# sphereisaiahmin-dev/sph-pie

Hardware: AMD Instinct MI355X
Metric: feeds/sec + sessions scanned/sec, 10^8 synthetic sessions, 1/2/4/8 MI355X (higher is better)
Workload: dtype int64

## Files before the change

include/pie_scan.h:

```cpp
#ifndef PIE_SCAN_H
#define PIE_SCAN_H

#include <stddef.h>
#include <stdint.h>

#ifdef __cplusplus
extern "C" {
#endif

#define PIE_ABI_VERSION 1

enum {
    PIE_OK = 0,
    PIE_E_INVAL = -1,
    PIE_E_NODEVICE = -2,
    PIE_E_HIP = -3,
    PIE_E_NOMEM = -4,
    PIE_E_CAPACITY = -5,
    PIE_E_STATE = -6
};

#define PIE_GEN_INTERVAL  1u
#define PIE_GEN_CLUSTERED 2u
#define PIE_GEN_TIME_ORDERED 4u
// ... 77 lines not shown
    uint64_t mask;
} pie_query;
int pie_scan_batch_begin(pie_ctx *ctx, const pie_query *queries, int n_q);
int pie_scan_batch_finish(pie_ctx *ctx, size_t *m_out);
int pie_scan_batch(pie_ctx *ctx, const pie_query *queries, int n_q, size_t *m_out);
int pie_batch_union_device_ptrs(pie_ctx *ctx, void **uoff_dev , void **rows_dev ,
                                void **mask_lo_dev , void **mask_hi_dev ,
                                size_t *mu_out);
int pie_batch_read_union(pie_ctx *ctx, int64_t *uoff_out, int32_t *rows_out, uint64_t *masks_out, size_t cap, size_t *mu_out);
#define PIE_WIDE_MAX 512
int pie_scan_wide_begin(pie_ctx *ctx, const pie_query *queries, int n_q);
int pie_scan_wide_finish(pie_ctx *ctx, size_t *m_out, size_t m_cap, int *n_q_out);
int pie_batch_union_wide_device_ptrs(pie_ctx *ctx, void **uoff_dev , void **rows_dev ,
                                     void **masks_dev , int *words_out, size_t *mu_out);
int pie_batch_read_union_wide(pie_ctx *ctx, int64_t *uoff_out, int32_t *rows_out, uint64_t *masks_out , size_t cap,
                              int *words_out, size_t *mu_out);
int pie_batch_pack_union_wide_device(pie_ctx *ctx, void *dst_i32, size_t u_pad, size_t cap);
int pie_scan_wide_begin_union(pie_ctx *ctx, const pie_query *queries, int n_q, void *msg_i32, size_t u_pad, size_t cap);
int pie_scan_wide_finish_packed(pie_ctx *ctx, size_t *m_out, size_t m_cap, int *n_q_out, int *ready_out);
int pie_set_batch_lanes(pie_ctx *ctx, int n_lanes);
int pie_batch_lanes(pie_ctx *ctx);
int pie_batch_room(pie_ctx *ctx);
int pie_scan_batch_flush(pie_ctx *ctx);
int pie_scan_batch_begin_union(pie_ctx *ctx, const pie_query *queries, int n_q, void *msg_i32, size_t u_pad, size_t cap);
int pie_scan_batch_begin_packed(pie_ctx *ctx, const pie_query *queries, int n_q, void *msg_i32, size_t msg_stride_words,
                                size_t u_pad, size_t idx_cap, void *counts_i32, size_t counts_stride_words);
int pie_scan_batch_finish_packed(pie_ctx *ctx, size_t *m_out, int *ready_out);
int pie_batch_read_results(pie_ctx *ctx, int qi, int32_t *counts_out, int64_t *offsets_out, int32_t *idx_out, size_t idx_cap,
                           size_t *m_out);
int pie_batch_result_device_ptrs(pie_ctx *ctx, int qi, void **counts_dev, void **offsets_dev, void **idx_dev);
int pie_batch_pack_union_device(pie_ctx *ctx, void *dst_i32, size_t u_pad, size_t cap);
int pie_batch_read_user_feed(pie_ctx *ctx, int qi, int32_t user, int32_t *idx_out, size_t idx_cap, size_t *k_out);

int pie_batch_fetch_requests(pie_ctx *ctx, const int32_t *qi, const int32_t *user, size_t n_req, size_t cap_rows, int64_t *req_off_out,
                             int32_t *idx_out, int64_t *start_out, int64_t *end_out, int32_t *disc_out, size_t *total_out);

int pie_read_results(pie_ctx *ctx, int32_t *counts_out, int64_t *offsets_out, int32_t *idx_out, size_t idx_cap,
                     size_t *m_out);
int pie_read_user_feed(pie_ctx *ctx, int32_t user, int32_t *idx_out, size_t idx_cap, size_t *k_out);
int pie_result_device_ptrs(pie_ctx *ctx, void **counts_dev, void **offsets_dev, void **idx_dev);
int pie_copy_results_device(pie_ctx *ctx, void *counts_dst, void *offsets_dst, void *idx_dst, size_t idx_cap);
int pie_pack_results_device(pie_ctx *ctx, void *dst_i32, size_t u_pad, size_t idx_cap);
int pie_fetch_rows(pie_ctx *ctx, const int32_t *idx, size_t m, int64_t *start, int64_t *end, int32_t *user,
                   int32_t *disc);

int pie_expired_queue(pie_ctx *ctx, int64_t prev_now, int64_t now, int32_t *queue_out, size_t cap, size_t *q_out);
// ... 231 lines not shown
```

sph-pie_amd/binding.py:

```python
import ctypes as C
import os

import numpy as np

from .build import HIP_LIB

PIE_GEN_INTERVAL = 1
PIE_GEN_CLUSTERED = 2
PIE_GEN_TIME_ORDERED = 4
PIE_END_NONE = -(2 ** 63)
INT64_MIN = -(2 ** 63)

PIE_E_CAPACITY = -5
PIE_E_STATE = -6
PIE_COMPACT_SHRINK = 1


class PieError(RuntimeError):
    def __init__(self, code, text):
        super().__init__("pie_scan error %d: %s" % (code, text))
        self.code = code


class PieTableInfo(C.Structure):
# ... 49 lines not shown
    ("pie_delete_users", C.c_int, [_P, _P, C.c_size_t, _P, C.c_size_t, C.POINTER(C.c_size_t), _P]),
    ("pie_delete_users_plan", C.c_int, [_P, C.c_size_t, C.c_int32, _P, _P]),
    ("pie_prune_before", C.c_int, [_P, C.c_int64, _P, C.c_size_t, C.POINTER(C.c_size_t)]),
    ("pie_retention_purge", C.c_int, [_P, C.c_int64, C.c_int32, C.c_int64, _P, C.c_size_t, C.POINTER(C.c_size_t)]),
    ("pie_retention_purge_tz", C.c_int, [_P, C.c_int64, C.c_int32, _P, _P, C.c_int32, _P, C.c_size_t, C.POINTER(C.c_size_t)]),
    ("pie_append_rows", C.c_int, [_P, _P, _P, _P, _P, C.c_size_t, C.c_int32]),
    ("pie_set_disciplines", C.c_int, [_P, C.c_uint64, C.c_int32]),
    ("pie_scan", C.c_int, [_P, C.c_int64, C.c_int64, _P, _P, _P, C.c_size_t, C.POINTER(C.c_size_t)]),
    ("pie_scan_device", C.c_int, [_P, C.c_int64, C.c_int64, C.POINTER(C.c_size_t)]),
    ("pie_scan_begin", C.c_int, [_P, C.c_int64, C.c_int64]),
    ("pie_scan_finish", C.c_int, [_P, C.POINTER(C.c_size_t)]),
    ("pie_scan_begin_packed", C.c_int, [_P, C.c_int64, C.c_int64, C.c_void_p, C.c_size_t, C.c_size_t]),
    ("pie_scan_finish_packed", C.c_int, [_P, C.POINTER(C.c_size_t), C.POINTER(C.c_int)]),
    ("pie_scan_begin_packed2", C.c_int, [_P, C.c_int64, C.c_int64, C.c_void_p, C.c_size_t, C.c_size_t, C.c_void_p]),
    ("pie_host_alloc", C.c_int, [_P, C.c_size_t, C.POINTER(_P), C.POINTER(_P)]),
    ("pie_host_free", C.c_int, [_P, _P]),
    ("pie_set_scan_form", C.c_int, [_P, C.c_int]),
    ("pie_set_ordered_run", C.c_int, [_P, C.c_int]),
    ("pie_set_wide_ordered", C.c_int, [_P, C.c_int]),
    ("pie_set_batch_lanes", C.c_int, [_P, C.c_int]),
    ("pie_batch_lanes", C.c_int, [_P]),
    ("pie_batch_room", C.c_int, [_P]),
    ("pie_scan_batch_flush", C.c_int, [_P]),
    ("pie_batch_pack_union_device", C.c_int, [_P, _P, C.c_size_t, C.c_size_t]),
    ("pie_table_info_get", C.c_int, [_P, C.POINTER(PieTableInfo)]),
    ("pie_hot_layout", C.c_int, [_P, _P, C.POINTER(C.c_int64), _P, _P, _P, C.c_size_t, _P, C.c_size_t]),
    ("pie_hot_order_key", C.c_uint64, [C.c_uint32, C.c_int32, C.c_uint32]),
    ("pie_hot_slot_bits", C.c_uint32, [C.c_uint32]),
    ("pie_scan_batch_begin", C.c_int, [_P, C.POINTER(PieQuery), C.c_int]),
    ("pie_scan_batch_finish", C.c_int, [_P, C.POINTER(C.c_size_t)]),
    ("pie_scan_batch", C.c_int, [_P, C.POINTER(PieQuery), C.c_int, C.POINTER(C.c_size_t)]),
    ("pie_scan_batch_begin_union", C.c_int, [_P, C.POINTER(PieQuery), C.c_int, C.c_void_p, C.c_size_t, C.c_size_t]),
    ("pie_batch_union_device_ptrs", C.c_int, [_P, C.POINTER(_P), C.POINTER(_P), C.POINTER(_P), C.POINTER(_P), C.POINTER(C.c_size_t)]),
    ("pie_batch_read_union", C.c_int, [_P, _P, _P, _P, C.c_size_t, C.POINTER(C.c_size_t)]),
    ("pie_scan_batch_begin_packed", C.c_int, [_P, C.POINTER(PieQuery), C.c_int, C.c_void_p, C.c_size_t, C.c_size_t, C.c_size_t, C.c_void_p, C.c_size_t]),
    ("pie_scan_batch_finish_packed", C.c_int, [_P, C.POINTER(C.c_size_t), C.POINTER(C.c_int)]),
    ("pie_scan_wide_begin", C.c_int, [_P, C.POINTER(PieQuery), C.c_int]),
    ("pie_scan_wide_finish", C.c_int, [_P, _P, C.c_size_t, C.POINTER(C.c_int)]),
    ("pie_batch_union_wide_device_ptrs", C.c_int, [_P, C.POINTER(_P), C.POINTER(_P), C.POINTER(_P), C.POINTER(C.c_int), C.POINTER(C.c_size_t)]),
    ("pie_batch_read_union_wide", C.c_int, [_P, _P, _P, _P, C.c_size_t, C.POINTER(C.c_int), C.POINTER(C.c_size_t)]),
    ("pie_batch_pack_union_wide_device", C.c_int, [_P, _P, C.c_size_t, C.c_size_t]),
    ("pie_scan_wide_begin_union", C.c_int, [_P, C.POINTER(PieQuery), C.c_int, _P, C.c_size_t, C.c_size_t]),
    ("pie_scan_wide_finish_packed", C.c_int, [_P, _P, C.c_size_t, C.POINTER(C.c_int), C.POINTER(C.c_int)]),
    ("pie_batch_mask_codes", C.c_int, [C.POINTER(PieQuery), C.c_int, _P, C.c_int32, _P, _P, _P, C.c_size_t, _P, _P]),
    ("pie_batch_read_results", C.c_int, [_P, C.c_int, _P, _P, _P, C.c_size_t, C.POINTER(C.c_size_t)]),
    ("pie_batch_result_device_ptrs", C.c_int, [_P, C.c_int, C.POINTER(_P), C.POINTER(_P), C.POINTER(_P)]),
# ... 379 lines not shown

    def scan_finish_packed(self):
        m, ready = C.c_size_t(0), C.c_int(0)
        rc = self._lib.pie_scan_finish_packed(self._ctx, C.byref(m), C.byref(ready))
        if self._begun and rc != -6:
            self._begun.pop(0)
        self._check(rc)
        return int(m.value), bool(ready.value)

    def scan_pipelined(self, k, now, cutoff):
        m = 0
        if k <= 0:
            return m
        self.scan_begin(now, cutoff)
        for i in range(k):
            if i + 1 < k:
                self.scan_begin(now, cutoff)
            m = self.scan_finish()
        return m

    _q_cache = None

    @staticmethod
    def _queries(queries):
        hit = PieScan._q_cache
        if hit is not None and hit[2] is queries and len(queries) == len(hit[0]):
            return hit[1]
        key = tuple(queries)
        if hit is not None and hit[0] == key:
            return hit[1]
        arr = (PieQuery * len(queries))()
        for k, (now, cutoff, mask) in enumerate(queries):
            arr[k].now, arr[k].cutoff, arr[k].mask = int(now), int(cutoff), int(mask) & (2 ** 64 - 1)
        PieScan._q_cache = (key, arr, queries)
        return arr

    def scan_batch_begin(self, queries):
        arr = self._queries(queries)
        self._check(self._lib.pie_scan_batch_begin(self._ctx, arr, len(queries)))
        self._batches = getattr(self, "_batches", [])
        self._batches.append(len(queries))

    def scan_batch_begin_packed(self, queries, msg_ptr, msg_stride, u_pad, idx_cap, counts_ptr=None, counts_stride=0):
        arr = self._queries(queries)
        self._check(self._lib.pie_scan_batch_begin_packed(self._ctx, arr, len(queries), msg_ptr, int(msg_stride), int(u_pad),
                                                          int(idx_cap), counts_ptr, int(counts_stride)))
        self._batches = getattr(self, "_batches", [])
        self._batches.append(len(queries))

    def scan_batch_begin_union(self, queries, msg_ptr, u_pad, cap):
        arr = self._queries(queries)
# ... 130 lines not shown
            if rc == PIE_E_CAPACITY and cap_rows is None and total.value > cap:
                cap = int(total.value)
                continue
            self._check(rc)
            break
        t = total.value
        return off, idx[:t], start[:t], end[:t], disc[:t]

    def batch_result_device_ptrs(self, qi):
        a, b, c = _P(), _P(), _P()
        self._check(self._lib.pie_batch_result_device_ptrs(self._ctx, int(qi), C.byref(a), C.byref(b), C.byref(c)))
        return a.value, b.value, c.value

    def set_batch_lanes(self, n_lanes):
        self._check(self._lib.pie_set_batch_lanes(self._ctx, int(n_lanes)))

    def batch_lanes(self):
        return int(self._lib.pie_batch_lanes(self._ctx))

    def batch_room(self):
        return int(self._lib.pie_batch_room(self._ctx))

    def scan_batch_pipelined(self, k, queries, depth=3):
        ms, begun, done = [], 0, 0
        depth = depth * self.batch_lanes()
        room = self._lib.pie_batch_room
        while done < k:
            while begun < k and begun - done < depth and room(self._ctx) > 0:
                self.scan_batch_begin(queries)
                begun += 1
                if begun == k:
                    self._check(self._lib.pie_scan_batch_flush(self._ctx))
            ms = self.scan_batch_finish()
            done += 1
        return ms

    def scan_batch_flush(self):
        self._check(self._lib.pie_scan_batch_flush(self._ctx))

    def result_device_ptrs(self):
        a, b, c = _P(), _P(), _P()
        self._check(self._lib.pie_result_device_ptrs(self._ctx, C.byref(a), C.byref(b), C.byref(c)))
        return a.value, b.value, c.value

    def copy_results_device(self, counts_ptr=None, offsets_ptr=None, idx_ptr=None, idx_cap=0):
        self._check(self._lib.pie_copy_results_device(self._ctx, counts_ptr, offsets_ptr, idx_ptr, int(idx_cap)))

    def pack_results_device(self, dst_ptr, u_pad, idx_cap):
        self._check(self._lib.pie_pack_results_device(self._ctx, dst_ptr, int(u_pad), int(idx_cap)))

    def fetch_rows(self, idx):
        idx = _col(idx, np.int32)
        m = idx.shape[0]
        s, e = np.empty(m, np.int64), np.empty(m, np.int64)
        u, d = np.empty(m, np.int32), np.empty(m, np.int32)
        self._check(self._lib.pie_fetch_rows(self._ctx, _ptr(idx), m, _ptr(s), _ptr(e), _ptr(u), _ptr(d)))
        return s, e, u, d

# ... 891 lines not shown
```

sph-pie_amd/build.py:

```python
import fcntl
import hashlib
import os
import shutil
import subprocess

PKG_DIR = os.path.dirname(os.path.abspath(__file__))
REPO = os.path.dirname(PKG_DIR)
CSRC = os.path.join(PKG_DIR, "csrc")
HIP_LIB = os.path.join(PKG_DIR, "libpie_hip.so")
UBENCH_LIB = os.path.join(PKG_DIR, "libpie_ubench.so")
NAPI_ADDON = os.path.join(PKG_DIR, "host", "pie_napi.node")
ORACLE_LIB = os.path.join(REPO, "oracle", "libpie_oracle.so")


def _digest(sources):
    h = hashlib.sha256()
    for path in sources:
        with open(path, "rb") as f:
            h.update(f.read())
    return h.hexdigest()


def _newer(target, sources):
    if not os.path.exists(target):
# ... 15 lines not shown
            return target
        tmp = "%s.tmp.%d" % (target, os.getpid())
        try:
            _run(make_cmd(tmp))
            os.replace(tmp, target)
            with open(target + ".srchash", "w") as f:
                f.write(_digest(sources))
        finally:
            if os.path.exists(tmp):
                os.remove(tmp)
    return target


def _run(cmd, cwd=None):
    res = subprocess.run(cmd, cwd=cwd, stdout=subprocess.PIPE, stderr=subprocess.STDOUT, text=True)
    if res.returncode != 0:
        raise RuntimeError("build step failed: %s\n%s" % (" ".join(cmd), res.stdout))
    return res.stdout


def build_hip(force=False):
    srcs = [os.path.join(CSRC, "pie_scan.hip"), os.path.join(CSRC, "pie_comm.hip"), os.path.join(CSRC, "pie_kernels.h"),
            os.path.join(CSRC, "pie_ordered.h"), os.path.join(CSRC, "pie_token.h"), os.path.join(CSRC, "pie_expq.h"), os.path.join(CSRC, "pie_expq_plan.h"),
            os.path.join(CSRC, "pie_turn_plan.h"), os.path.join(CSRC, "pie_wait.h"), os.path.join(REPO, "include", "pie_scan.h")]
    hipcc = shutil.which("hipcc") or "/opt/rocm/bin/hipcc"
    return _build(HIP_LIB, srcs, lambda out: [hipcc, "-O3", "-std=c++17", "--offload-arch=gfx950", "-fPIC", "-shared",
                                              "-o", out, os.path.join(CSRC, "pie_scan.hip"), os.path.join(CSRC, "pie_comm.hip"),
                                              "-ldl"], force)


def build_ubench(force=False):
    src = os.path.join(CSRC, "pie_ubench.hip")
    hipcc = shutil.which("hipcc") or "/opt/rocm/bin/hipcc"
    return _build(UBENCH_LIB, [src], lambda out: [hipcc, "-O3", "-std=c++17", "--offload-arch=gfx950", "-fPIC", "-shared", "-o", out, src], force)


def build_oracle(force=False):
    odir = os.path.join(REPO, "oracle")
    srcs = [os.path.join(odir, "pie_oracle.c"), os.path.join(odir, "pie_oracle.h")]
    return _build(ORACLE_LIB, srcs, lambda out: ["make", "-C", odir, "-B", "libpie_oracle.so", "OUT=" + out], force)


def build_napi(force=False):
    src = os.path.join(CSRC, "pie_napi.c")
    if not os.path.exists(src):
        return None
    inc = None
# ... 16 lines not shown
```

sph-pie_amd/csrc/pie_scan.hip:

```cpp
#include "../../include/pie_scan.h"
#include "pie_kernels.h"
#include "pie_ordered.h"
#include "pie_token.h"
#include "pie_turn_plan.h"
#include "pie_expq.h"
#include "pie_wait.h"

#include <hip/hip_runtime.h>

#include <cstring>
#include <rocprim/device/device_radix_sort.hpp>
#include <rocprim/device/device_scan.hpp>

#include <cstdarg>
#include <cstddef>
#include <cstdio>
#include <cstdlib>
#include <algorithm>
#include <cstring>
#include <ctime>
#include <string>
#include <vector>

#include <fcntl.h>
#include <sys/mman.h>
#include <sys/stat.h>
#include <unistd.h>
// ... 202 lines not shown
    int n_cus = 0;
    hipStream_t own_stream = nullptr;
    hipStream_t stream = nullptr;
    unsigned long long seq_counter = 0;
    char err[512] = "";

    long long n = 0;
    int n_users = 0;
    long long cap_rows = 0;
    long long sel_cap = 0;
    int cap_users = 0;
    long long *d_start = nullptr, *d_end = nullptr;
    int *d_user = nullptr, *d_disc = nullptr;
    lkey_t* d_key = nullptr;
    PayRec* d_pay = nullptr;
    fkey_t* d_fkey = nullptr;
    long long fkey_base = 0;
    int fkey_shift = 0;
    bool fkey_poor = false;
    unsigned int* d_hist = nullptr;
    std::vector<unsigned int> key_hist;
    std::vector<unsigned long long> key_hist_above;
    long long key_hist_rows = 0;
    long long key_base = 0;
    int key_shift = 0;
    bool key_ok = false;
    bool key_dirty = false;
    bool key_poor = false;
    bool key_rebuild = false;
    bool keyed_enabled = true;
    int order_block = 512;
    bool no_ride = false;
    bool no_fused_order = false;
    int k1_keyed = 0xC85;
    long long* d_range = nullptr;
    char* h_stage = nullptr;
    char* d_stage = nullptr;
    size_t stage_bytes = 0;
    bool expired_copy_total = false;
    struct AsyncStage { char* h = nullptr; char* d = nullptr; size_t bytes = 0; hipEvent_t ev = nullptr; bool pending = false; } astage[2];
    int astage_next = 0;
    bool async_mutations = true;
    std::vector<uint8_t> set_end_keep;
    std::vector<size_t> set_end_slots;
    int* d_shard_rows = nullptr;
    int* d_shard_users = nullptr;
// ... 192 lines not shown
    bool profiling = false;
    std::vector<ScanEvents> ring;
    int ring_used = 0;
    double k1_ms_sum = 0, scan_ms_sum = 0;
    unsigned n_profiled = 0;
};

namespace {

int fail(pie_ctx* c, int code, const char* fmt, ...)
{
    va_list ap;
    va_start(ap, fmt);
    if (c) vsnprintf(c->err, sizeof c->err, fmt, ap);
    else vsnprintf(g_create_error, sizeof g_create_error, fmt, ap);
    va_end(ap);
    return code;
}

#ifdef PIE_HOST_PROF
struct HostProf {
    double acc[16] = {0};
    unsigned long long n[16] = {0};
    timespec last{};
    void start() { clock_gettime(CLOCK_MONOTONIC, &last); }
    void tick(int i)
    {
        timespec t{};
        clock_gettime(CLOCK_MONOTONIC, &t);
        acc[i] += (double)(t.tv_sec - last.tv_sec) * 1e6 + (double)(t.tv_nsec - last.tv_nsec) * 1e-3;
        n[i]++;
        last = t;
    }
    void report() const
    {
        static const char* names[16] = {"begin: checks + dense test", "begin: slot / span set-up", "begin: tables", "begin: launch", "begin: rest",
                                        "finish: k2 launch", "finish: wait", "finish: rest", "", "", "", "", "", "", "", ""};
        for (int i = 0; i < 8; ++i)
            if (n[i]) fprintf(stderr, "[pie host prof] %-28s %8.3f us x %llu\n", names[i], acc[i] / (double)n[i], n[i]);
    }
};
HostProf g_prof;
#define PIE_PROF_START() g_prof.start()
#define PIE_PROF_TICK(i) g_prof.tick(i)
#else
#define PIE_PROF_START() ((void)0)
#define PIE_PROF_TICK(i) ((void)0)
#endif

#define PIE_HIP(c, call)                                                                              \
    do {                                                                                              \
        hipError_t e_ = (call);                                                                       \
        if (e_ != hipSuccess)                                                                         \
            return fail((c), e_ == hipErrorOutOfMemory ? PIE_E_NOMEM : PIE_E_HIP, "%s: %s (%s:%d)", #call, \
                        hipGetErrorString(e_), __FILE__, __LINE__);                                   \
    } while (0)

template <class T>
void dfree(T*& p)
{
    if (p) (void)hipFree(p);
    p = nullptr;
}

DirectSlots direct_of(const pie_ctx* c, const Slot& sl);

Slot* oldest_in_flight(pie_ctx* c)
{
    if (c->n_flight == 0) return nullptr;
    return &c->slot[c->n_flight == 2 ? c->next_slot : (c->next_slot ^ 1)];
// ... 619 lines not shown
    }
    *out = &a;
    return PIE_OK;
}

int validate_users(pie_ctx* c, long long row0 = 0)
{
    if (c->n - row0 <= 0) return PIE_OK;
    PIE_HIP(c, hipMemsetAsync(c->d_summary, 0, sizeof(Summary), c->stream));
    const int grid = c->n_cus * 8;
    hipLaunchKernelGGL(k_validate_users, dim3(grid), dim3(256), 0, c->stream, c->d_user + row0, c->n - row0, c->n_users,
                       &c->d_summary->bad_rows);
    PIE_HIP(c, hipGetLastError());
    PIE_HIP(c, hipMemcpyAsync(c->h_summary, c->d_summary, sizeof(Summary), hipMemcpyDeviceToHost, c->stream));
    PIE_HIP(c, hipStreamSynchronize(c->stream));
    if (c->h_summary->bad_rows)
        return fail(c, PIE_E_INVAL, "%u rows carry a user id outside [0, %d)", c->h_summary->bad_rows, c->n_users);
    return PIE_OK;
}

int build_keys(pie_ctx* c, long long row0, bool rebuild = false)
{
    c->hix.valid = false;
    if (!c->d_key || !c->d_pay || !c->d_fkey) { c->key_ok = false; return PIE_OK; }
    const bool write_pay = !(rebuild && c->key_ok);
    if (c->n == 0) { c->key_ok = true; c->key_base = 0; c->key_shift = 0; c->key_dirty = false; return PIE_OK; }
    hipStream_t s = c->stream;
    const int grid = c->n_cus * 8;
    const bool full_build = row0 == 0 || !c->key_ok || rebuild;
    if (full_build && !(rebuild && c->key_ok && c->ord.valid && c->ord.rows == c->n)) ord_invalidate(c);
    timespec tb0{};
    if (full_build) {
        const int land_rc = expq_land(c, "key build");
        if (land_rc) return land_rc;
        PIE_HIP(c, hipStreamSynchronize(s));
        clock_gettime(CLOCK_MONOTONIC, &tb0);
    }
    if (row0 == 0 || !c->key_ok || rebuild) {
        const long long init[2] = {INT64_MAX, INT64_MIN};
        long long got[2];
        PIE_HIP(c, hipMemcpyAsync(c->d_range, init, sizeof init, hipMemcpyHostToDevice, s));
        hipLaunchKernelGGL(k_end_range, dim3(grid), dim3(256), 0, s, c->d_end, c->n, c->d_range);
        PIE_HIP(c, hipGetLastError());
        PIE_HIP(c, hipMemcpyAsync(got, c->d_range, sizeof got, hipMemcpyDeviceToHost, s));
        PIE_HIP(c, hipStreamSynchronize(s));
        c->key_base = 0;
// ... 1502 lines not shown

int lane_after_mutation(pie_ctx* c, int lane)
{
    if (lane == 0 || c->lane_mut_epoch[lane] == c->mut_epoch) return PIE_OK;
    PIE_HIP(c, hipStreamWaitEvent(lane_stream_of(c, lane), c->mut_event, 0));
    c->lane_mut_epoch[lane] = c->mut_epoch;
    return PIE_OK;
}

void take_spans(pie_ctx* c, BatchSlot& b)
{
    char** const lane_spans = c->bspan + b.lane * 3;
    b.span = lane_spans[c->lane_span_next[b.lane]];
    c->lane_span_next[b.lane] = (c->lane_span_next[b.lane] + 1) % 3;
    b.zero_span = lane_spans[(c->lane_span_next[b.lane] + 1) % 3];
}

BatchSlot* waiting_tail(pie_ctx* c, int lane)
{
    BatchSlot& prev = lane_slot(c, lane, 1);
    return c->lane_flight[lane] >= 1 && prev.in_flight && prev.k2_pending && !prev.ordered ? &prev : nullptr;
}

int batch_begin(pie_ctx* c, const pie_query* qs, int n_q, int msg_kind, int* msg, long long msg_stride, int u_pad, long long msg_cap,
                int* msg_counts, long long msg_counts_stride)
{
    PIE_PROF_START();
    int rc = begin_checks(c, qs, n_q, kBatchMax, "a batch");
    if (rc) return rc;
    const bool ord_batch = batch_supported(c) && ordered_batch_wanted(c) && !c->ord_lists_only;
    bool unsupported = !ord_batch && (!batch_supported(c) || c->key_poor || c->batch_poor);
    unsigned char dense_q[kBatchMax];
    bool fine = false;
    if (!unsupported && !classify_queries(c, qs, n_q, dense_q, &fine)) unsupported = true;
    int lane = 0;
    rc = pick_lane(c, ord_batch ? 1 : c->n_lanes, &lane);
    if (rc) return rc;
    BatchSlot& b = lane_slot(c, lane);
    claim_slot(c, b, lane, n_q, unsupported, msg_kind, msg, msg_stride, u_pad, msg_cap, msg_counts, msg_counts_stride);
    b.wide = false;
    for (int q = 0; q < n_q; ++q) { b.q[q] = qs[q]; b.fallback[q] = unsupported || dense_q[q]; b.idx_of[q] = nullptr; b.list_ok[q] = false; }
    hipStream_t s = b.stream;
    PIE_PROF_TICK(0);
    if (unsupported) {
        begin_fallback_only(c, b);
        return PIE_OK;
    }
    rc = regrow_union_buckets(c);
    if (rc) return rc;
    rc = ord_batch ? PIE_OK : ensure_batch(c, lane);
    if (rc) return rc;
    if (fine && !ord_batch && c->hix.enabled && !c->hix.valid && c->b_flight == 0) {
        rc = hot_build(c);
        if (rc) return rc;
    }
    rc = order_lane_after_main(c, lane);
    if (rc) return rc;
// ... 37 lines not shown
        return PIE_OK;
    }
    take_spans(c, b);
    b.seq = ++c->bseq_counter;
    const int plan = fine ? 3 : 2;
    b.k1_blocks = c->plan_blocks[plan];
    c->scans_begun++;
    const bool ride = other && !c->no_ride;
    if (other && !ride) launch_batch_k2(c, *other, s);
    if (b.ev_index >= 0) PIE_HIP(c, hipEventRecord(c->ring[b.ev_index].e0, s));
    PIE_PROF_TICK(1);
#define PIE_BATCH_RIDE(KT, HI)                                                                                          \
    hipLaunchKernelGGL((k_scan_batch_with_tail<8, true, KT, HI>), dim3((unsigned)(b.k1_blocks + t.tiles)), dim3(kK1Threads), 0, s, a, t)
#define PIE_BATCH(KT, KEYPTR, KEYFN, IMPOSSIBLE)                                                                         \
    do {                                                                                                                \
        BatchScanArgs<KT> a;                                                                                            \
        a.pay = c->d_pay; a.end = c->d_end; a.key = KEYPTR; a.n = c->n; a.rows_per_block = c->plan_rows[plan];          \
        a.n_users = c->n_users; a.n_q = n_q; a.dshift = c->bdshift;                                                     \
        a.counts = reinterpret_cast<int*>(b.span);                                                                      \
        a.summary = reinterpret_cast<Summary*>(b.span + span_counts_bytes(c) + span_tiles_bytes(c) + span_parts_bytes() + 128); \
        a.direct = b.direct; a.mtab = b.mtab; a.run_shift = c->run_shift;                                               \
        unsigned nk[kBatchMax];                                                                                         \
        unsigned mk = IMPOSSIBLE;                                                                                       \
        for (int q = 0; q < n_q; ++q) {                                                                                 \
            nk[q] = KEYFN(c, qs[q].now);                                                                                \
            if (!b.fallback[q] && nk[q] < mk) mk = nk[q];                                                               \
        }                                                                                                               \
        a.min_key = mk;                                                                                                 \
        a.hot = nullptr; a.hot_lo = a.hot_main = 0; a.hot_delta_n = nullptr; a.hot_delta_cap = 0;                       \
        if (b.hot && mk >= 1 && mk <= kFineKeyMax) {  \
            a.hot = c->hix.rec; a.hot_lo = c->hix.off[mk]; a.hot_main = c->hix.n_main;                                  \
            a.hot_delta_n = c->hix.delta_n; a.hot_delta_cap = (unsigned)c->hix.delta_cap;                               \
            const long long recs = a.hot_main - a.hot_lo + c->hix.delta_bound;                                          \
            const long long per = (long long)c->hix.recs_per_thread * kK1Threads;                                      \
            const long long want = (recs + per - 1) / per;                                                              \
            b.k1_blocks = (int)(want < 1 ? 1 : want < b.k1_blocks ? want : b.k1_blocks);                                \
        }                                                                                                               \
        fill_batch_tables(c, b, qs, nk, a.tab);                                                                         \
        PIE_PROF_TICK(2);                                                                                               \
        if (ride) {                                                                                                     \
            UnionTailArgs t;                                                                                            \
            fill_tail_args(c, *other, t);                                                                               \
            if (t.n_q > 32) PIE_BATCH_RIDE(KT, true);                                                                   \
            else PIE_BATCH_RIDE(KT, false);                                                                             \
            other->k2_pending = false;                                                                                  \
        } else {                                                                                                        \
            hipLaunchKernelGGL((k_scan_batch<8, true, KT>), dim3((unsigned)b.k1_blocks), dim3(kK1Threads), 0, s, a);    \
        }                                                                                                               \
    } while (0)
    if (fine) PIE_BATCH(fkey_t, c->d_fkey, host_fine_key_of, 0xFFu);
    else PIE_BATCH(lkey_t, c->d_key, host_key_of, 0xFFFFu);
#undef PIE_BATCH
#undef PIE_BATCH_RIDE
    PIE_PROF_TICK(3);
    PIE_HIP(c, hipGetLastError());
    if (b.ev_index >= 0) PIE_HIP(c, hipEventRecord(c->ring[b.ev_index].e1, s));
    b.k2_pending = true;
    b.in_flight = true;
    batch_begun(c, lane);
    PIE_PROF_TICK(4);
    return PIE_OK;
// ... 125 lines not shown
{
    if (b.list_ok[qi]) return PIE_OK;
    return batch_materialize(c, b, &qi, 1);
}

int batch_pack_union(pie_ctx* c, BatchSlot& b, void* dst_i32, size_t u_pad, size_t cap);

int batch_finish(pie_ctx* c, int* ready_out)
{
    if (ready_out) *ready_out = 0;
    BatchSlot* bp = oldest_batch(c);
    if (!bp) return fail(c, PIE_E_STATE, "pie_scan_batch_finish without pie_scan_batch_begin");
    if (bp->wide) return fail(c, PIE_E_STATE, "the oldest batch in flight is wide: finish it with pie_scan_wide_finish");
    BatchSlot& b = *bp;
    hipStream_t s = b.stream ? b.stream : c->stream;
    bool all_ready = true;
    PIE_PROF_START();
    if (!b.unsupported) {
        if (b.k2_pending) {
            launch_batch_k2(c, b, s);
            PIE_HIP(c, hipGetLastError());
        }
        PIE_PROF_TICK(5);
        const WaitResult w = word_wait(c, &b.bh->seq, b.seq, [&] { return hipStreamQuery(s); }, 1000.0, kPaceSummary);
        if (w.end != WaitEnd::Ready) {
            batch_left(c, b);
            if (w.end == WaitEnd::Failed) return fail(c, PIE_E_HIP, "batched scan failed: %s", hipGetErrorString((hipError_t)w.err));
            return fail(c, PIE_E_HIP, "batch summary not published within %.0f ms (PIE_WAIT_DEADLINE_MS): kernel hung?", w.waited_ms);
        }
        PIE_PROF_TICK(6);
        bool overflow = false;
        {
            const Summary us = b.bh->s;
            b.mu = us.m;
            overflow = us.n_over > 0 || us.bad_rows > 0;
            for (int q = 0; q < b.n_q; ++q) {
                b.last[q] = us;
                b.last[q].m = b.bh->mq[q];
                if (overflow) b.fallback[q] = true;
            }
            if (us.n_over > 0 && b.ordered) c->ord_lists_only = true;
            else if (us.n_over > 0) {
                if (c->bdshift < kUnionShiftMax) c->bdshift_want = c->bdshift + 1;
                else c->batch_poor = true;
            }
            b.union_part = !overflow;
// ... 560 lines not shown
    if (const char* v = getenv("PIE_EXPIRED_COPY_TOTAL")) c->expired_copy_total = atoi(v) != 0;
    if (const char* v = getenv("PIE_ASYNC_MUTATIONS")) c->async_mutations = atoi(v) != 0;
    if (const char* v = getenv("PIE_HOT_INDEX")) c->hix.enabled = atoi(v) != 0;
    if (const char* v = getenv("PIE_HOT_RECS")) { const int r = atoi(v); if (r == 1 || r == 2 || r == 4) c->hix.recs_per_thread = r; }
    if (const char* v = getenv("PIE_HOT_ORDER")) { if (!strcmp(v, "row")) c->hix.order = 0; else if (!strcmp(v, "slot")) c->hix.order = 1; }
    if (const char* v = getenv("PIE_BATCH_LANES")) { const int l = atoi(v); if (l >= 0 && l <= kLaneMax) c->lanes_want = l; }
    if (const char* v = getenv("PIE_ORDER_BLOCK")) { const int b = atoi(v); if (b == 256 || b == 512 || b == 1024) c->order_block = b; }
    if (const char* v = getenv("PIE_RUN_SHIFT")) { const int r = atoi(v); if (r >= 0 && r <= 3) { c->run_shift = r; c->run_shift_pinned = true; } }
    if (const char* v = getenv("PIE_ORDERED")) { const int m = atoi(v); if (m >= 0 && m <= 2) c->ord.mode = m; }
    if (const char* v = getenv("PIE_WIDE_ORDERED")) c->wide_ordered = atoi(v) == 1;
    if (const char* v = getenv("PIE_ORD_GRID")) { const int g = atoi(v); if (g >= 1 && g <= 64) c->ord.grid_mult = g; }
    if (const char* v = getenv("PIE_WAIT_DEADLINE_MS")) { const double d = atof(v); if (d > 0) c->wait_deadline_ms = d; }
    if (const char* v = getenv("PIE_EXPQ_BLOCKS_PER_CU")) { const int g = atoi(v); if (g >= 1 && g <= 16) c->expq.blocks_per_cu = g; }
    if (const char* v = getenv("PIE_EXPQ_MAX_BLOCKS")) { const int g = atoi(v); if (g >= 1) c->expq.max_blocks = g; }
    if (const char* v = getenv("PIE_K1_KEYED")) {
        const int k = (int)strtol(v, nullptr, 0);
        c->keyed_enabled = k != 0;
        if (k & 0x400) c->k1_keyed = k;
    }
    *ctx_out = c;
    return PIE_OK;
}

int pie_ctx_destroy(pie_ctx* c)
{
    if (!c) return PIE_OK;
#ifdef PIE_HOST_PROF
    g_prof.report();
#endif
    (void)hipSetDevice(c->device);
    (void)side_passes_land(c, "pie_ctx_destroy");
    (void)hipStreamSynchronize(c->stream);
    free_table(c);
    dfree(c->d_shard_rows);
    dfree(c->d_shard_users);
    cmp_forget(c);
    token_drop(c);
    dfree(c->tokx.status);
    dfree(c->tokx.d_stage);
    if (c->tokx.h_stage) (void)hipHostFree(c->tokx.h_stage);
    if (c->tokx.turn_done) (void)hipEventDestroy(c->tokx.turn_done);
    for (hipEvent_t e : c->tokx.ev)
        if (e) (void)hipEventDestroy(e);
    side_close(c->tokx.side);
    for (auto& l : c->tokx.lk) {
        if (l.h) (void)hipHostFree(l.h);
// ... 791 lines not shown
    return batch_begin(c, queries, n_q, 0, nullptr, 0, 0, 0, nullptr, 0);
}

int pie_scan_batch_begin_packed(pie_ctx* c, const pie_query* queries, int n_q, void* msg_i32, size_t msg_stride_words, size_t u_pad,
                                size_t idx_cap, void* counts_i32, size_t counts_stride_words)
{
    if (!c) return PIE_E_INVAL;
    if (!msg_i32 || u_pad < (size_t)c->n_users || u_pad > 0x7FFFFFF0u || msg_stride_words < u_pad + 2 + idx_cap)
        return fail(c, PIE_E_INVAL, "bad message destination / u_pad < n_users / stride below u_pad + 2 + idx_cap");
    if (counts_i32 && counts_stride_words < (size_t)c->n_users) return fail(c, PIE_E_INVAL, "counts stride below n_users");
    PIE_HIP(c, hipSetDevice(c->device));
    return batch_begin(c, queries, n_q, 1, (int*)msg_i32, (long long)msg_stride_words, (int)u_pad, (long long)idx_cap, (int*)counts_i32,
                       (long long)counts_stride_words);
}

int pie_scan_batch_begin_union(pie_ctx* c, const pie_query* queries, int n_q, void* msg_i32, size_t u_pad, size_t cap)
{
    if (!c) return PIE_E_INVAL;
    if (!msg_i32 || u_pad < (size_t)c->n_users || u_pad > 0x7FFFFFF0u) return fail(c, PIE_E_INVAL, "bad union destination / u_pad < n_users");
    PIE_HIP(c, hipSetDevice(c->device));
    return batch_begin(c, queries, n_q, 2, (int*)msg_i32, 0, (int)u_pad, (long long)cap, nullptr, 0);
}

int pie_scan_batch_flush(pie_ctx* c)
{
    if (!c) return PIE_E_INVAL;
    PIE_HIP(c, hipSetDevice(c->device));
    for (int lane = 0; lane < kLaneMax; ++lane) {
        for (int age = c->lane_flight[lane]; age >= 1; --age) {
            BatchSlot& b = c->bslot[lane * kBatchSlots + (c->lane_next[lane] + kBatchSlots - age) % kBatchSlots];
            if (b.in_flight && b.k2_pending && !b.ordered && !b.unsupported) launch_batch_k2(c, b, b.stream ? b.stream : c->stream);
        }
    }
    PIE_HIP(c, hipGetLastError());
    return PIE_OK;
}

int pie_scan_batch_finish_packed(pie_ctx* c, size_t* m_out, int* ready_out)
{
    if (!c) return PIE_E_INVAL;
    PIE_HIP(c, hipSetDevice(c->device));
    int rc = batch_finish(c, ready_out);
    if (rc) return rc;
    if (m_out)
        for (int q = 0; q < c->bres->n_q; ++q) m_out[q] = (size_t)c->bres->last[q].m;
    return PIE_OK;
}

int pie_scan_batch_finish(pie_ctx* c, size_t* m_out) { return pie_scan_batch_finish_packed(c, m_out, nullptr); }

int pie_scan_batch(pie_ctx* c, const pie_query* queries, int n_q, size_t* m_out)
{
    if (!c) return PIE_E_INVAL;
    if (c->b_flight) return fail(c, PIE_E_STATE, "a batch is in flight: finish it first");
    int rc = pie_scan_batch_begin(c, queries, n_q);
    if (rc) return rc;
    return pie_scan_batch_finish(c, m_out);
// ... 3115 lines not shown
```

Before: 491.1 billion.

## Run pipelined batch bursts in native code and cache per-burst query tables

```diff
diff --git a/include/pie_scan.h b/include/pie_scan.h
--- a/include/pie_scan.h
+++ b/include/pie_scan.h
@@ -123,6 +123,7 @@
 int pie_batch_lanes(pie_ctx *ctx);
 int pie_batch_room(pie_ctx *ctx);
 int pie_scan_batch_flush(pie_ctx *ctx);
+int pie_scan_batch_run(pie_ctx *ctx, const pie_query *queries, int n_q, int k, int depth_per_lane, size_t *m_out);
 int pie_scan_batch_begin_union(pie_ctx *ctx, const pie_query *queries, int n_q, void *msg_i32, size_t u_pad, size_t cap);
 int pie_scan_batch_begin_packed(pie_ctx *ctx, const pie_query *queries, int n_q, void *msg_i32, size_t msg_stride_words,
                                 size_t u_pad, size_t idx_cap, void *counts_i32, size_t counts_stride_words);
diff --git a/sph-pie_amd/binding.py b/sph-pie_amd/binding.py
--- a/sph-pie_amd/binding.py
+++ b/sph-pie_amd/binding.py
@@ -95,6 +95,7 @@
     ("pie_batch_lanes", C.c_int, [_P]),
     ("pie_batch_room", C.c_int, [_P]),
     ("pie_scan_batch_flush", C.c_int, [_P]),
+    ("pie_scan_batch_run", C.c_int, [_P, C.POINTER(PieQuery), C.c_int, C.c_int, C.c_int, C.POINTER(C.c_size_t)]),
     ("pie_batch_pack_union_device", C.c_int, [_P, _P, C.c_size_t, C.c_size_t]),
     ("pie_table_info_get", C.c_int, [_P, C.POINTER(PieTableInfo)]),
     ("pie_hot_layout", C.c_int, [_P, _P, C.POINTER(C.c_int64), _P, _P, _P, C.c_size_t, _P, C.c_size_t]),
@@ -520,11 +521,11 @@
     _q_cache = None
 
     @staticmethod
-    def _queries(queries):
+    def _queries(queries, by_identity=True):
         hit = PieScan._q_cache
-        if hit is not None and hit[2] is queries and len(queries) == len(hit[0]):
+        if by_identity and hit is not None and hit[2] is queries and len(queries) == len(hit[0]):
             return hit[1]
-        key = tuple(queries)
+        key = tuple(map(tuple, queries))
         if hit is not None and hit[0] == key:
             return hit[1]
         arr = (PieQuery * len(queries))()
@@ -701,18 +702,16 @@
         return int(self._lib.pie_batch_room(self._ctx))
 
     def scan_batch_pipelined(self, k, queries, depth=3):
-        ms, begun, done = [], 0, 0
-        depth = depth * self.batch_lanes()
-        room = self._lib.pie_batch_room
-        while done < k:
-            while begun < k and begun - done < depth and room(self._ctx) > 0:
-                self.scan_batch_begin(queries)
-                begun += 1
-                if begun == k:
-                    self._check(self._lib.pie_scan_batch_flush(self._ctx))
-            ms = self.scan_batch_finish()
-            done += 1
-        return ms
+        if k <= 0:
+            return []
+        nq = len(queries)
+        old = getattr(self, "_batches", [])
+        rc = self._lib.pie_scan_batch_run(self._ctx, self._queries(queries, False), nq, int(k), int(depth), self._m_buf)
+        fifo = old + [nq] * k
+        self._batches = fifo[k:] if rc == 0 else ([] if not old or rc != -1 else old)
+        if rc:
+            self._check(rc)
+        return self._m_buf[:fifo[k - 1]]
 
     def scan_batch_flush(self):
         self._check(self._lib.pie_scan_batch_flush(self._ctx))
diff --git a/sph-pie_amd/build.py b/sph-pie_amd/build.py
--- a/sph-pie_amd/build.py
+++ b/sph-pie_amd/build.py
@@ -61,7 +61,7 @@
 def build_hip(force=False):
     srcs = [os.path.join(CSRC, "pie_scan.hip"), os.path.join(CSRC, "pie_comm.hip"), os.path.join(CSRC, "pie_kernels.h"),
             os.path.join(CSRC, "pie_ordered.h"), os.path.join(CSRC, "pie_token.h"), os.path.join(CSRC, "pie_expq.h"), os.path.join(CSRC, "pie_expq_plan.h"),
-            os.path.join(CSRC, "pie_turn_plan.h"), os.path.join(CSRC, "pie_wait.h"), os.path.join(REPO, "include", "pie_scan.h")]
+            os.path.join(CSRC, "pie_turn_plan.h"), os.path.join(CSRC, "pie_burst_plan.h"), os.path.join(CSRC, "pie_wait.h"), os.path.join(REPO, "include", "pie_scan.h")]
     hipcc = shutil.which("hipcc") or "/opt/rocm/bin/hipcc"
     return _build(HIP_LIB, srcs, lambda out: [hipcc, "-O3", "-std=c++17", "--offload-arch=gfx950", "-fPIC", "-shared",
                                               "-o", out, os.path.join(CSRC, "pie_scan.hip"), os.path.join(CSRC, "pie_comm.hip"),
diff --git a/sph-pie_amd/csrc/pie_burst_plan.h b/sph-pie_amd/csrc/pie_burst_plan.h
--- /dev/null
+++ b/sph-pie_amd/csrc/pie_burst_plan.h
@@ -0,0 +1,36 @@
+#ifndef PIE_BURST_PLAN_H
+#define PIE_BURST_PLAN_H
+
+namespace pie {
+
+enum class BurstOp { Begin, Flush, Finish, Done };
+
+struct BurstPlan {
+    int k, window;
+    int begun = 0, done = 0;
+    bool flush_due = false;
+
+    BurstPlan(int k_, int depth_per_lane, int lanes) : k(k_), window(depth_per_lane * lanes) {}
+
+    bool asks_room() const { return !flush_due && done < k && begun < k && begun - done < window; }
+
+    BurstOp next(int room)
+    {
+        if (flush_due) {
+            flush_due = false;
+            return BurstOp::Flush;
+        }
+        if (done >= k) return BurstOp::Done;
+        if (begun < k && begun - done < window && room > 0) {
+            ++begun;
+            flush_due = begun == k;
+            return BurstOp::Begin;
+        }
+        ++done;
+        return BurstOp::Finish;
+    }
+};
+
+}
+
+#endif
diff --git a/sph-pie_amd/csrc/pie_scan.hip b/sph-pie_amd/csrc/pie_scan.hip
--- a/sph-pie_amd/csrc/pie_scan.hip
+++ b/sph-pie_amd/csrc/pie_scan.hip
@@ -3,6 +3,7 @@
 #include "pie_ordered.h"
 #include "pie_token.h"
 #include "pie_turn_plan.h"
+#include "pie_burst_plan.h"
 #include "pie_expq.h"
 #include "pie_wait.h"
 
@@ -251,6 +252,7 @@
     std::vector<unsigned int> key_hist;
     std::vector<unsigned long long> key_hist_above;
     long long key_hist_rows = 0;
+    unsigned long long key_builds = 0;
     long long key_base = 0;
     int key_shift = 0;
     bool key_ok = false;
@@ -489,8 +491,10 @@
 struct HostProf {
     double acc[16] = {0};
     unsigned long long n[16] = {0};
+    unsigned long long finishes = 0, finishes_waited = 0;
     timespec last{};
     void start() { clock_gettime(CLOCK_MONOTONIC, &last); }
+    void finish_looked(bool landed) { finishes++; finishes_waited += landed ? 0 : 1; }
     void tick(int i)
     {
         timespec t{};
@@ -505,14 +509,17 @@
                                         "finish: k2 launch", "finish: wait", "finish: rest", "", "", "", "", "", "", "", ""};
         for (int i = 0; i < 8; ++i)
             if (n[i]) fprintf(stderr, "[pie host prof] %-28s %8.3f us x %llu\n", names[i], acc[i] / (double)n[i], n[i]);
+        if (finishes) fprintf(stderr, "[pie host prof] %-28s %llu of %llu\n", "finish: had to wait", finishes_waited, finishes);
     }
 };
 HostProf g_prof;
 #define PIE_PROF_START() g_prof.start()
 #define PIE_PROF_TICK(i) g_prof.tick(i)
+#define PIE_PROF_FINISH_LOOKED(landed) g_prof.finish_looked(landed)
 #else
 #define PIE_PROF_START() ((void)0)
 #define PIE_PROF_TICK(i) ((void)0)
+#define PIE_PROF_FINISH_LOOKED(landed) ((void)0)
 #endif
 
 #define PIE_HIP(c, call)                                                                              \
@@ -1178,6 +1185,7 @@
 int build_keys(pie_ctx* c, long long row0, bool rebuild = false)
 {
     c->hix.valid = false;
+    c->key_builds++;
     if (!c->d_key || !c->d_pay || !c->d_fkey) { c->key_ok = false; return PIE_OK; }
     const bool write_pay = !(rebuild && c->key_ok);
     if (c->n == 0) { c->key_ok = true; c->key_base = 0; c->key_shift = 0; c->key_dirty = false; return PIE_OK; }
@@ -2726,8 +2734,35 @@
     return c->lane_flight[lane] >= 1 && prev.in_flight && prev.k2_pending && !prev.ordered ? &prev : nullptr;
 }
 
+struct BurstTables {
+    struct Seen {
+        unsigned long long key_builds;
+        long long n, key_hist_rows, key_base, fkey_base;
+        int n_q, n_disc, key_shift, fkey_shift, k1_keyed, bdshift_want;
+        bool key_dirty, key_poor, fkey_poor, batch_poor, ord_lists_only, hot_valid;
+        bool operator==(const Seen& o) const
+        {
+            return key_builds == o.key_builds && n == o.n && key_hist_rows == o.key_hist_rows && key_base == o.key_base && fkey_base == o.fkey_base &&
+                   n_q == o.n_q && n_disc == o.n_disc && key_shift == o.key_shift && fkey_shift == o.fkey_shift && k1_keyed == o.k1_keyed &&
+                   bdshift_want == o.bdshift_want && key_dirty == o.key_dirty && key_poor == o.key_poor && fkey_poor == o.fkey_poor &&
+                   batch_poor == o.batch_poor && ord_lists_only == o.ord_lists_only && hot_valid == o.hot_valid;
+        }
+    };
+    static Seen look(const pie_ctx* c, int n_q)
+    {
+        return Seen{c->key_builds, c->n, c->key_hist_rows, c->key_base, c->fkey_base, n_q, c->n_disc, c->key_shift, c->fkey_shift, c->k1_keyed,
+                    c->bdshift_want, c->key_dirty, c->key_poor, c->fkey_poor, c->batch_poor, c->ord_lists_only, c->hix.valid};
+    }
+    bool classified = false, have_tab = false;
+    Seen seen{};
+    bool any = false, fine = false;
+    unsigned char dense[kBatchMax];
+    unsigned min_key = 0;
+    BatchTables tab;
+};
+
 int batch_begin(pie_ctx* c, const pie_query* qs, int n_q, int msg_kind, int* msg, long long msg_stride, int u_pad, long long msg_cap,
-                int* msg_counts, long long msg_counts_stride)
+                int* msg_counts, long long msg_counts_stride, BurstTables* pre = nullptr)
 {
     PIE_PROF_START();
     int rc = begin_checks(c, qs, n_q, kBatchMax, "a batch");
@@ -2736,7 +2771,22 @@
     bool unsupported = !ord_batch && (!batch_supported(c) || c->key_poor || c->batch_poor);
     unsigned char dense_q[kBatchMax];
     bool fine = false;
-    if (!unsupported && !classify_queries(c, qs, n_q, dense_q, &fine)) unsupported = true;
+    if (pre && !(pre->classified && pre->seen == BurstTables::look(c, n_q))) pre->classified = pre->have_tab = false;
+    if (!unsupported && pre && pre->classified) {
+        memcpy(dense_q, pre->dense, (size_t)n_q);
+        fine = pre->fine;
+        if (!pre->any) unsupported = true;
+    } else if (!unsupported) {
+        const bool any = classify_queries(c, qs, n_q, dense_q, &fine);
+        if (pre) {
+            pre->seen = BurstTables::look(c, n_q);
+            pre->classified = true;
+            pre->any = any;
+            pre->fine = fine;
+            memcpy(pre->dense, dense_q, (size_t)n_q);
+        }
+        if (!any) unsupported = true;
+    }
     int lane = 0;
     rc = pick_lane(c, ord_batch ? 1 : c->n_lanes, &lane);
     if (rc) return rc;
@@ -2820,10 +2870,13 @@
         a.direct = b.direct; a.mtab = b.mtab; a.run_shift = c->run_shift;                                               \
         unsigned nk[kBatchMax];                                                                                         \
         unsigned mk = IMPOSSIBLE;                                                                                       \
-        for (int q = 0; q < n_q; ++q) {                                                                                 \
-            nk[q] = KEYFN(c, qs[q].now);                                                                                \
-            if (!b.fallback[q] && nk[q] < mk) mk = nk[q];                                                               \
-        }                                                                                                               \
+        const bool have_tab = pre && pre->have_tab;    \
+        if (have_tab) mk = pre->min_key;                                                                                \
+        else                                                                                                            \
+            for (int q = 0; q < n_q; ++q) {                                                                             \
+                nk[q] = KEYFN(c, qs[q].now);                                                                            \
+                if (!b.fallback[q] && nk[q] < mk) mk = nk[q];                                                           \
+            }                                                                                                           \
         a.min_key = mk;                                                                                                 \
         a.hot = nullptr; a.hot_lo = a.hot_main = 0; a.hot_delta_n = nullptr; a.hot_delta_cap = 0;                       \
         if (b.hot && mk >= 1 && mk <= kFineKeyMax) {  \
@@ -2834,7 +2887,15 @@
             const long long want = (recs + per - 1) / per;                                                              \
             b.k1_blocks = (int)(want < 1 ? 1 : want < b.k1_blocks ? want : b.k1_blocks);                                \
         }                                                                                                               \
-        fill_batch_tables(c, b, qs, nk, a.tab);                                                                         \
+        if (have_tab) a.tab = pre->tab;                                                                                 \
+        else {                                                                                                          \
+            fill_batch_tables(c, b, qs, nk, a.tab);                                                                     \
+            if (pre && pre->classified) {                                                                               \
+                pre->min_key = mk;                                                                                      \
+                pre->tab = a.tab;                                                                                       \
+                pre->have_tab = true;                                                                                   \
+            }                                                                                                           \
+        }                                                                                                               \
         PIE_PROF_TICK(2);                                                                                               \
         if (ride) {                                                                                                     \
             UnionTailArgs t;                                                                                            \
@@ -3006,6 +3067,7 @@
             PIE_HIP(c, hipGetLastError());
         }
         PIE_PROF_TICK(5);
+        PIE_PROF_FINISH_LOOKED(b.bh->seq == b.seq);
         const WaitResult w = word_wait(c, &b.bh->seq, b.seq, [&] { return hipStreamQuery(s); }, 1000.0, kPaceSummary);
         if (w.end != WaitEnd::Ready) {
             batch_left(c, b);
@@ -3612,6 +3674,14 @@
     return PIE_OK;
 }
 
+#ifdef PIE_HOST_PROF
+void pie_host_prof_report(int reset)
+{
+    g_prof.report();
+    if (reset) g_prof = HostProf{};
+}
+#endif
+
 int pie_ctx_destroy(pie_ctx* c)
 {
     if (!c) return PIE_OK;
@@ -4449,10 +4519,8 @@
     return batch_begin(c, queries, n_q, 2, (int*)msg_i32, 0, (int)u_pad, (long long)cap, nullptr, 0);
 }
 
-int pie_scan_batch_flush(pie_ctx* c)
-{
-    if (!c) return PIE_E_INVAL;
-    PIE_HIP(c, hipSetDevice(c->device));
+static int batch_flush(pie_ctx* c)
+{
     for (int lane = 0; lane < kLaneMax; ++lane) {
         for (int age = c->lane_flight[lane]; age >= 1; --age) {
             BatchSlot& b = c->bslot[lane * kBatchSlots + (c->lane_next[lane] + kBatchSlots - age) % kBatchSlots];
@@ -4460,6 +4528,57 @@
         }
     }
     PIE_HIP(c, hipGetLastError());
+    return PIE_OK;
+}
+
+int pie_scan_batch_flush(pie_ctx* c)
+{
+    if (!c) return PIE_E_INVAL;
+    PIE_HIP(c, hipSetDevice(c->device));
+    return batch_flush(c);
+}
+
+int pie_scan_batch_run(pie_ctx* c, const pie_query* queries, int n_q, int k, int depth_per_lane, size_t* m_out)
+{
+    if (!c) return PIE_E_INVAL;
+    if (!queries || n_q < 1 || n_q > kBatchMax) return fail(c, PIE_E_INVAL, "a batch holds 1..%d queries (got %d)", kBatchMax, n_q);
+    if (k < 1 || depth_per_lane < 1) return fail(c, PIE_E_INVAL, "a burst runs k >= 1 batches, depth >= 1 per lane (got k = %d, depth = %d)", k, depth_per_lane);
+    PIE_HIP(c, hipSetDevice(c->device));
+    BurstTables pre;
+    BurstPlan plan(k, depth_per_lane, c->n_lanes);
+    int rc = PIE_OK, ours = 0, theirs = c->b_flight;
+    auto finish_oldest = [&]() {
+        const int flight = c->b_flight;
+        const int r = batch_finish(c, nullptr);
+        if (c->b_flight < flight) --(theirs > 0 ? theirs : ours);
+        return r;
+    };
+    for (;;) {
+        const BurstOp op = plan.next(plan.asks_room() ? pie_batch_room(c) : 0);
+        if (op == BurstOp::Done) break;
+        if (op == BurstOp::Begin) {
+            rc = batch_begin(c, queries, n_q, 0, nullptr, 0, 0, 0, nullptr, 0, &pre);
+            if (rc == PIE_OK) ++ours;
+        } else if (op == BurstOp::Flush) {
+            rc = batch_flush(c);
+        } else {
+            rc = finish_oldest();
+        }
+        if (rc) break;
+    }
+    if (rc) {
+        char first[sizeof c->err];
+        memcpy(first, c->err, sizeof first);
+        while (ours > 0 && c->b_flight > 0) {
+            const int flight = c->b_flight;
+            (void)finish_oldest();
+            if (c->b_flight >= flight) break;
+        }
+        memcpy(c->err, first, sizeof first);
+        return rc;
+    }
+    if (m_out)
+        for (int q = 0; q < c->bres->n_q; ++q) m_out[q] = (size_t)c->bres->last[q].m;
     return PIE_OK;
 }
 
```

Result: no change. 490.5 billion (-0.1%).
